# petitioner/MOAI-FHE-TransformerInference-Public

Hardware: AMD Instinct MI355X
Metric: NTT+INTT algorithmic GB/s (N=2^16, L=44x60-bit, batch=256 ciphertexts/GPU) vs HBM peak (higher is better)
Workload: dtype u64; 1 GPU; configs[1]: negacyclic NTT then INTT, N=65536, 44 x 60-bit primes, 256 ciphertexts x 2 polys per GPU; batch_per_gpu=256, batch_total=256, coeff_modulus=CoeffModulus::Create(65536, 44 x 60), bytes_per_coeff_per_transform=16

## Files before the change

moai-fhe-transformerinference-public_amd/csrc/launch.h:

```cpp
#pragma once
#include <type_traits>

#include "common.h"

namespace moai {

#define MOAI_KNOBS(X)                                                                                                          \
    X(NTT_FP, 1, "0: primes below 2^51 stay on the integer units in every transform, key switch and mod-down")                \
    X(NTT_LAZY8, 1, "0: integer primes below 2^60 take the exact butterflies instead of the approximate Shoup quotient")       \
    X(NTT_LDSTW, 1, "0: the forward contiguous pass loads its first stages' twiddles from memory instead of through LDS")      \
    X(NTT_CHUNK_MB, 0, "> 0: launch the two passes of a transform per chunk of polynomials of at most this many MiB")          \
    X(NTT_NAIVE, 0, "1: one launch per radix-2 stage over global memory (cross-check path)")                                   \
    X(NTT_COOP, 0, "1: the single-launch persistent transform (N >= 4096)")                                                    \
    X(NTT_COOP_WPC, 4, "single-launch transform: workgroups per compute unit")                                                 \
    X(NTT_COOP_DELAY, 4, "single-launch transform: rows a second pass stays behind the first")                                 \
    X(NTT_COOP_OCC, 4, "single-launch transform: occupancy the kernel is compiled for (3 or 4)")                               \
    X(KS_FP_MIN_ROWS, 16, "batch * L from which the key switch uses the FP64 arithmetic modes")                                \
    X(KS_TMP_MB, 8192, "MiB of key-switch digits in flight: sets how many output moduli share a launch")                       \
    X(KS_P1_ITEMS, 8, "1: the key switch's strided pass at N = 2^16 runs one tile per workgroup instead of eight, pipelined")  \
    X(KS_P1_PRE, 0, "1: the M_FPN strided pass of the key switch takes its twiddles as plain doubles")                         \
    X(KS_MAC_PF, 1, "key residues of the FP64 key-switch MAC: 0 loaded next to their use, 1 at its head, 2 at the digit's head") \
    X(KS_HOIST_PAIR, 4, "rotations per pass of the hoisted MAC in the FP64 modes: 4, 2, or 0 for one")                         \
    X(MD_FP_MIN_ROWS, 256, "polynomials * L from which mod-down and rescale use the FP64 arithmetic modes")                    \
    X(MATMUL_FP, 1, "0: moai_ct_pt_matmul keeps primes below 2^51 on the integer kernel")                                      \
    X(DEC_TMP_MB, 1024, "MiB of scratch per chunk of moai_ckks_decode when the stream's arena is smaller")

enum Knob
{
#define MOAI_KNOB_ID(id, dflt, what) K_##id,
    MOAI_KNOBS(MOAI_KNOB_ID)
#undef MOAI_KNOB_ID
    KNOB_COUNT
// ... 63 lines not shown
```

moai-fhe-transformerinference-public_amd/csrc/modarith.hip.h:

```cpp
#pragma once
#include "common.h"

namespace moai {

__device__ __forceinline__ uint64_t mulhi64(uint64_t a, uint64_t b)
{
    return __umul64hi(a, b);
}

__device__ __forceinline__ uint64_t mul_shoup_lazy(uint64_t y, uint64_t w, uint64_t wq, uint64_t q)
{
    uint64_t t = mulhi64(y, wq);
    return y * w + t * (0 - q);
}

__device__ __forceinline__ uint64_t csub(uint64_t x, uint64_t m)
{
    return x >= m ? x - m : x;
}

__device__ __forceinline__ uint64_t barrett128(uint64_t lo, uint64_t hi, uint64_t q, uint64_t cr0, uint64_t cr1)
{
    uint64_t carry = mulhi64(lo, cr0);
    uint64_t t_lo = lo * cr1;
// ... 77 lines not shown
__device__ __forceinline__ void fold2(uint64_t &lx, uint64_t &hx, uint64_t &ly, uint64_t &hy, uint64_t q, uint64_t cr0, uint64_t cr1)
{
    seed2(lx, hx, ly, hy, reduce2(lx, hx, ly, hy, q, cr0, cr1));
}

__device__ __forceinline__ void ct_bfly(uint64_t &x, uint64_t &y, uint64_t w, uint64_t wq, uint64_t q, uint64_t q2)
{
    uint64_t u = csub(x, q2);
    uint64_t v = mul_shoup_lazy(y, w, wq, q);
    x = u + v;
    y = u + q2 - v;
}

__device__ __forceinline__ void ct_bfly_noguard(uint64_t &x, uint64_t &y, uint64_t w, uint64_t wq, uint64_t q, uint64_t q2)
{
    uint64_t v = mul_shoup_lazy(y, w, wq, q);
    uint64_t u = x;
    x = u + v;
    y = u + q2 - v;
}

enum
{
    M_LAZY8 = -2,
    M_GUARD2 = -1,
    M_GUARD = 0,
    M_NOGUARD = 1,
    M_FPN = 2,
    M_FPR = 3
};

__device__ __forceinline__ double u2d(uint64_t b)
{
    return __longlong_as_double((long long)b);
}
__device__ __forceinline__ uint64_t d2u(double d)
{
    return (uint64_t)__double_as_longlong(d);
}
__device__ __forceinline__ double fp_from_u64(uint64_t v)
{
    return __builtin_fma((double)(uint32_t)(v >> 32), 4294967296.0, (double)(uint32_t)v);
}
__device__ __forceinline__ double fp_from_u52(uint64_t v)
{
    return u2d(v | 0x4330000000000000ull) - 4503599627370496.0;
// ... 91 lines not shown
    const uint32_t hi = (uint32_t)(p >> 32) + y0 * w1 + y1 * w0 + t0 * n1 + t1 * n0;
    return ((uint64_t)hi << 32) | (uint32_t)p;
}
__device__ __forceinline__ void ct_bfly_lazy8(uint64_t &x, uint64_t &y, uint64_t w, uint64_t wq, uint64_t nq, uint64_t n4q)
{
    const uint64_t u = csub_sign(x, n4q);
    const uint64_t v = mul_shoup_approx(y, w, wq, nq);
    x = u + v;
    y = u - (v + n4q);
}

__device__ __forceinline__ void gs_bfly_lazy8(uint64_t &x, uint64_t &y, uint64_t w, uint64_t wq, uint64_t nq, uint64_t n4q)
{
    const uint64_t u = x, v = y;
    x = csub_sign(u + v, n4q);
    y = mul_shoup_approx(u - (v + n4q), w, wq, nq);
}
__device__ __forceinline__ void gs_bfly_last_lazy8(uint64_t &x, uint64_t &y, const Tw &ninv, const Tw &ninv_w1, uint64_t nq, uint64_t n4q)
{
    const uint64_t u = x, v = y;
    x = mul_shoup_approx(u + v, ninv.w, ninv.wq, nq);
    y = mul_shoup_approx(u - (v + n4q), ninv_w1.w, ninv_w1.wq, nq);
}
template <bool LZ>
__device__ __forceinline__ void gs_bfly_sel(uint64_t &x, uint64_t &y, uint64_t w, uint64_t wq, uint64_t a, uint64_t b);

template <int MODE, int STAGES_LEFT = 0>
__device__ __forceinline__ void ct_bfly_t(uint64_t &x, uint64_t &y, uint64_t w, uint64_t wq, uint64_t q, uint64_t q2)
{
    if (MODE == M_LAZY8)
    {
        ct_bfly_lazy8(x, y, w, wq, q, q2);
    }
    else if (MODE == M_GUARD2)
    {
        ct_bfly_guard2<(STAGES_LEFT % 2) == 0>(x, y, w, wq, q, q2);
    }
    else if (MODE == M_FPN)
    {
        ct_bfly_fp<false>(x, y, w, wq, q, q2);
    }
    else if (MODE == M_FPR)
    {
        ct_bfly_fp<true>(x, y, w, wq, q, q2);
    }
    else if (MODE == M_NOGUARD)
// ... 83 lines not shown
```

moai-fhe-transformerinference-public_amd/csrc/ntt.hip:

```cpp
#include "ntt_kernels.hip.h"
#include "launch.h"

namespace moai {

bool noguard_ok(uint64_t q)
{
    return q < (~0ull) / 36;
}

int ntt_mode(const moai_ctx *c, uint32_t prime, bool allow_fp)
{
    const int m = (int)c->pc_host[prime].fp_mode;
    if (allow_fp && m && tuning(K_NTT_FP))
    {
        return m;
    }
    return noguard_ok(c->primes[prime]) ? M_NOGUARD : M_GUARD;
}

TwPair twiddles(const moai_ctx *c, int mode, bool inverse)
{
    if (mode >= M_FPN)
    {
        return inverse ? TwPair{ c->inv_twf, c->inv_twfb } : TwPair{ c->fwd_twf, c->fwd_twfb };
// ... 9 lines not shown
    a.tw = t.tw;
    a.twb = t.twb;
    a.pc = c->pc;
    a.rows = rows;
    for (size_t r = 0; r < MOAI_MAX_RNS; ++r)
    {
        a.sel.idx[r] = (uint32_t)(r < L ? r : 0);
        a.selp.idx[r] = rows.idx[r < L ? r : 0];
    }
    a.Lsel = (uint32_t)L;
    a.L = (uint32_t)L;
    a.n_poly = (uint32_t)n_poly;
    a.total_work = 0;
    a.src = nullptr;
    a.src_stride = a.src_off = 0;
    a.lds_twiddles = tuning(K_NTT_LDSTW) ? 1u : 0u;
    return a;
}

static bool lazy8_ok(const moai_ctx *c, uint32_t prime)
{
    return tuning(K_NTT_LAZY8) && c->primes[prime] < (1ull << 60);
}

template <int LOGN, int MODE>
static void launch_fwd_mode(const moai_ctx *c, NttArgs a, hipStream_t s)
{
    constexpr uint32_t tpr = 1u << (LOGN - 12);
    a.total_work = a.n_poly * a.Lsel * tpr;
    const TwPair t = twiddles(c, MODE, false);
    a.tw = t.tw;
    a.twb = t.twb;
    hipLaunchKernelGGL((ntt_fwd_strided<LOGN, MODE>), dim3(a.total_work), dim3(256), 0, s, a);
    hipLaunchKernelGGL((ntt_fwd_contig<LOGN, MODE>), dim3(a.total_work), dim3(256), 0, s, a);
}

template <int LOGN>
static int launch_fwd(const moai_ctx *c, const NttArgs &base, hipStream_t s)
{
    for (int mode : { M_LAZY8, M_GUARD2, M_NOGUARD, M_FPN, M_FPR })
    {
        NttArgs a = base;
        a.Lsel = 0;
        for (uint32_t r = 0; r < a.L; ++r)
        {
            const uint32_t prime = a.rows.idx[r];
            int m = ntt_mode(c, prime);
            if (m == M_GUARD)
            {
                m = lazy8_ok(c, prime) ? M_LAZY8 : M_GUARD2;
            }
            if (m == mode)
            {
                a.selp.idx[a.Lsel] = prime;
                a.sel.idx[a.Lsel++] = r;
            }
        }
        if (a.Lsel == 0)
        {
            continue;
        }
        MOAI_TRY((dispatch<M_LAZY8, M_GUARD2, M_NOGUARD, M_FPN, M_FPR>("forward transform mode ", mode, [&](auto MD) {
            launch_fwd_mode<LOGN, decltype(MD)::value>(c, a, s);
            return MOAI_OK;
        })));
    }
    return MOAI_OK;
}

template <int LOGN, int IM>
static void launch_inv_class(NttArgs a, hipStream_t s)
{
    constexpr uint32_t tpr = 1u << (LOGN - 12);
    if (!a.Lsel)
    {
        return;
    }
    a.total_work = a.n_poly * a.Lsel * tpr;
    hipLaunchKernelGGL((ntt_inv_contig<LOGN, IM>), dim3(a.total_work), dim3(256), 0, s, a);
    hipLaunchKernelGGL((ntt_inv_strided<LOGN, IM>), dim3(a.total_work), dim3(256), 0, s, a);
}

template <int LOGN>
static void launch_inv(const moai_ctx *c, const NttArgs &base, hipStream_t s)
{
    NttArgs cls[4] = { base, base, base, base };
    for (NttArgs &a : cls)
    {
        a.Lsel = 0;
    }
    const TwPair fp = twiddles(c, M_FPN, true);
    cls[2].tw = cls[3].tw = fp.tw;
    cls[2].twb = cls[3].twb = fp.twb;
    for (uint32_t r = 0; r < base.L; ++r)
    {
        const uint32_t prime = base.rows.idx[r];
        const int m = ntt_mode(c, prime);
        NttArgs &dst = m == M_FPN ? cls[2] : (m == M_FPR ? cls[3] : (lazy8_ok(c, prime) ? cls[1] : cls[0]));
        dst.selp.idx[dst.Lsel] = prime;
        dst.sel.idx[dst.Lsel++] = r;
    }
    launch_inv_class<LOGN, 0>(cls[0], s);
    launch_inv_class<LOGN, 1>(cls[1], s);
    launch_inv_class<LOGN, 2>(cls[2], s);
    launch_inv_class<LOGN, 3>(cls[3], s);
}

static size_t coop_grid(const moai_ctx *c)
{
    const long wpc = tuning(K_NTT_COOP_WPC);
    return (size_t)c->num_cu * (size_t)(wpc > 0 ? wpc : 4);
}

static uint32_t coop_delay()
{
    const long d = tuning(K_NTT_COOP_DELAY);
    return (uint32_t)(d > 0 ? d : 1);
}

static size_t coop_steps_cap(const moai_ctx *c, size_t rows)
{
    return rows + coop_delay() + coop_grid(c) + 8;
}

static size_t coop_state_bytes(const moai_ctx *c, size_t rows)
{
    return sizeof(CoopState) + sizeof(uint32_t) * (rows + 8 * coop_steps_cap(c, rows));
}
// ... 212 lines not shown
```

moai-fhe-transformerinference-public_amd/csrc/ntt_kernels.hip.h:

```cpp
#pragma once
#include "modarith.hip.h"

namespace moai {

__device__ __forceinline__ uint32_t xcd_remap(uint32_t b, uint32_t total)
{
    if (total & 7u)
    {
        return b;
    }
    return (b & 7u) * (total >> 3) + (b >> 3);
}

__device__ __forceinline__ void lds_barrier()
{
    asm volatile("s_waitcnt lgkmcnt(0)\n\ts_barrier" ::: "memory");
}

__device__ __forceinline__ void lds_wave_sync()
{
    asm volatile("s_waitcnt lgkmcnt(0)" ::: "memory");
}

__device__ __forceinline__ uint32_t phys_contig(uint32_t e)
// ... 12 lines not shown
    }
    return e;
}

struct NttArgs
{
    uint64_t *data;
    const Tw *tw;
    const Tw *twb;
    const PrimeConst *pc;
    RowMap rows;
    RowMap sel;
    RowMap selp;
    uint32_t L;
    uint32_t Lsel;
    uint32_t n_poly;
    uint32_t total_work;
    const uint64_t *src;
    uint32_t src_stride;
    uint32_t src_off;
    uint32_t lds_twiddles;
};

template <int MODE>
__device__ __forceinline__ uint64_t mode_q(const PrimeConst &pc)
{
    return MODE >= M_FPN ? pc.qd : (MODE == M_LAZY8 ? pc.nq : pc.q);
}
template <int MODE>
__device__ __forceinline__ uint64_t mode_q2(const PrimeConst &pc)
{
    return MODE >= M_FPN ? pc.qinv : (MODE == M_LAZY8 ? pc.n4q : pc.q2);
}

struct LoadIdentity
{
    __device__ __forceinline__ uint64_t operator()(uint64_t v) const
    {
        return v;
    }
};

struct LoadBarrett
{
    uint64_t q, cr1;
    __device__ __forceinline__ uint64_t operator()(uint64_t v) const
    {
        return barrett64(v, q, cr1);
    }
};

struct LoadFp
{
    uint64_t qd, qinv;
    __device__ __forceinline__ uint64_t operator()(uint64_t v) const
// ... 1 lines not shown
        return d2u(fp_red(fp_from_u64(v), u2d(qd), u2d(qinv)));
    }
};

struct LoadFp52
{
    uint64_t qd, qinv;
    __device__ __forceinline__ uint64_t operator()(uint64_t v) const
    {
        return d2u(fp_red(fp_from_u52(v), u2d(qd), u2d(qinv)));
    }
};

struct LoadBarrettFp
{
    uint64_t q, cr1, qd, qinv;
    __device__ __forceinline__ uint64_t operator()(uint64_t v) const
    {
        return d2u(fp_red(fp_from_u52(barrett64(v, q, cr1)), u2d(qd), u2d(qinv)));
    }
};


template <int MODE>
__device__ __forceinline__ void ct_bfly_stage(uint64_t &x, uint64_t &y, uint64_t w, uint64_t wq, uint64_t q, uint64_t q2, int stages_left)
{
    if (MODE == M_GUARD2)
    {
        if (stages_left & 1)
        {
            ct_bfly_guard2<false>(x, y, w, wq, q, q2);
        }
        else
        {
            ct_bfly_guard2<true>(x, y, w, wq, q, q2);
        }
    }
    else
    {
        ct_bfly_t<MODE>(x, y, w, wq, q, q2);
    }
}

template <int LOGN>
__device__ __forceinline__ void strided_load_raw(const uint64_t *__restrict__ irow, const uint32_t tid, uint64_t (&raw)[16])
{
    constexpr int GB = 12 - (LOGN - 8);
    constexpr uint32_t G = 1u << GB;
#pragma unroll
    for (int j = 0; j < 16; ++j)
// ... 10 lines not shown
{
    typedef const Tw __attribute__((address_space(4))) *TwConst;
    const TwConst twa = (TwConst)(uintptr_t)tw;
    constexpr int R1 = LOGN - 8;
    constexpr int RB = R1 - 4;
    constexpr int GB = 12 - R1;
    constexpr uint32_t G = 1u << GB;
#ifdef MOAI_DIAG_NOCOMPUTE
    const int diag_stages = (q == 0x7ff8dead0000beefull) ? 4 : 0;
#define MOAI_DIAG_STAGE_OK(u) && ((u) < diag_stages)
#else
#define MOAI_DIAG_STAGE_OK(u)
#endif
#pragma unroll
    for (int u = 0; u < 4; ++u)
    {
        const int half = 8 >> u;
#pragma unroll
        for (int j = 0; j < 16; ++j)
        {
            if (!(j & half) MOAI_DIAG_STAGE_OK(u))
            {
                const uint32_t ti = (1u << u) + (uint32_t)(j >> (4 - u));
                ct_bfly_stage<MODE>(x[j], x[j + half], twa[ti].w, twa[ti].wq, q, q2, LOGN - 1 - u);
            }
        }
    }
    if (RB > 0)
    {
        double twb[16];
        if (PRE)
        {
            const uint32_t thp = tid >> GB;
#pragma unroll
            for (int s = 4; s < R1; ++s)
            {
                const int cnt = 16 >> (R1 - s);
#pragma unroll
                for (int i = 0; i < cnt; ++i)
                {
                    twb[cnt - 1 + i] = tw1[(1u << s) + ((thp << (4 - (R1 - s))) | (uint32_t)i)];
                }
            }
        }
        if (SYNC_FIRST)
        {
            lds_barrier();
// ... 8 lines not shown
        const uint32_t th = tid >> GB;
#pragma unroll
        for (int j = 0; j < 16; ++j)
        {
            x[j] = lds[phys_strided<GB>((th << (GB + 4)) | ((uint32_t)j << GB) | g)];
        }
#pragma unroll
        for (int s = 4; s < R1; ++s)
        {
            const int half = 1 << (R1 - 1 - s);
#pragma unroll
            for (int j = 0; j < 16; ++j)
            {
                if (!(j & half) MOAI_DIAG_STAGE_OK(s - 4))
                {
                    if (PRE)
                    {
                        ct_bfly_fp1<MODE == M_FPR>(x[j], x[j + half], twb[(16 >> (R1 - s)) - 1 + (j >> (R1 - s))], u2d(q), u2d(q2));
                    }
                    else
                    {
                        uint32_t t_ = (th << 4) | (uint32_t)j;
                        Tw t = LDSTW ? ldstw[(1u << s) + (t_ >> (R1 - s))] : tw[(1u << s) + (t_ >> (R1 - s))];
                        ct_bfly_stage<MODE>(x[j], x[j + half], t.w, t.wq, q, q2, LOGN - 1 - s);
                    }
                }
            }
        }
#pragma unroll
        for (int j = 0; j < 16; ++j)
        {
            uint32_t t_ = (th << 4) | (uint32_t)j;
#ifdef MOAI_DIAG_NOSTORE
            if (x[j] == 0x7ff8dead0000beefull)
#endif
            row[(t_ << 8) + g] = x[j];
        }
    }
    else
    {
#pragma unroll
        for (int j = 0; j < 16; ++j)
        {
            uint32_t e = (uint32_t)j * 256u + tid;
            row[((e >> GB) << 8) + (e & (G - 1))] = x[j];
        }
    }
// ... 40 lines not shown
#pragma unroll 1
    for (uint32_t it = 0; it < (uint32_t)ITEMS; ++it)
    {
        uint32_t t = tid;
        asm volatile("" : "+v"(t));
        const bool more = it + 1u < (uint32_t)ITEMS;
        if (more)
        {
            strided_load_raw<LOGN>(inp + (tile0 + it + 1u) * G, t, raw);
        }
        strided_core<LOGN, MODE, false, true, true>(x, rowp + (tile0 + it) * G, tw, q, q2, lds, t, nullptr, ldstw);
        if (more)
        {
#pragma unroll
            for (int j = 0; j < 16; ++j)
            {
                x[j] = op(raw[j]);
            }
        }
    }
}

template <int LOGN, int MODE = M_GUARD>
__global__ __launch_bounds__(256, (MODE == M_GUARD2 || MODE == M_LAZY8 || MODE == M_FPR || MODE == M_NOGUARD) ? 4 : 5) void ntt_fwd_strided(NttArgs a)
{
    constexpr uint32_t TPR = 1u << (LOGN - 12);
    constexpr bool LDSTW = LOGN == 16 && (MODE == M_GUARD2 || MODE == M_LAZY8 || MODE == M_FPR || MODE == M_NOGUARD);
    __shared__ uint64_t lds[4096 + (LDSTW ? 512 : 0)];
    const uint32_t w = xcd_remap(blockIdx.x, a.total_work);
    const uint32_t tile = w % TPR;
    const uint32_t srow = w / TPR;
    const uint32_t si = srow % a.Lsel;
    const uint32_t r = __builtin_amdgcn_readfirstlane(a.sel.idx[si]);
    const uint32_t prime = __builtin_amdgcn_readfirstlane(a.selp.idx[si]);
    const PrimeConst &pc = a.pc[prime];
    uint64_t *rowp = a.data + ((size_t)((srow / a.Lsel) * a.L + r) << LOGN);
    if (MODE >= M_FPN)
    {
        LoadFp op;
        op.qd = pc.qd;
        op.qinv = pc.qinv;
        fwd_strided_tile<LOGN, LoadFp, MODE, false, LDSTW>(rowp, rowp, tile, a.tw + ((size_t)prime << LOGN), pc.qd, pc.qinv, lds, threadIdx.x, op);
    }
    else
    {
        fwd_strided_tile<LOGN, LoadIdentity, MODE, false, LDSTW>(rowp, rowp, tile, a.tw + ((size_t)prime << LOGN), mode_q<MODE>(pc), mode_q2<MODE>(pc),
                                                                 lds, threadIdx.x);
    }
}

struct StoreTile
{
    ulonglong2 *out;
    __device__ __forceinline__ void fetch(const uint32_t (&)[4])
    {
    }
    __device__ __forceinline__ void operator()(int, uint32_t ch, ulonglong2 v) const
    {
        out[ch] = v;
    }
};

template <int LOGN, int MODE = M_GUARD, class StoreOp = StoreTile>
__device__ __forceinline__ void fwd_contig_tile(uint64_t *__restrict__ rowp, uint32_t tile, const Tw *__restrict__ tw,
                                                uint64_t q, uint64_t q2, ulonglong2 *lds2, const uint32_t tid,
                                                const Tw *__restrict__ twb, uint64_t cr1, StoreOp store, Tw *ldstw = nullptr)
{
    constexpr int R1 = LOGN - 8;
    uint64_t *lds = reinterpret_cast<uint64_t *>(lds2);
    uint64_t *__restrict__ base = rowp + ((size_t)tile << 12);
    const uint32_t b = tid >> 4;
    const uint32_t tl = tid & 15u;
    const uint32_t blk = (tile << 4) + b;
    const Tw *__restrict__ twbt = twb + (size_t)tile * (15 * 256);

    if (ldstw)
    {
        const uint32_t lane = tid & 63u;
        if (lane < 60u)
        {
            const uint32_t bb = ((tid >> 6) << 2) + lane / 15u, i = lane % 15u;
            const uint32_t u = i == 0 ? 0u : (i < 3 ? 1u : (i < 7 ? 2u : 3u)), k = i - ((1u << u) - 1u);
            ldstw[bb * 15u + i] = tw[(1u << (R1 + u)) + (((tile << 4) + bb) << u) + k];
        }
    }
    uint64_t x[16];
#pragma unroll
    for (int j = 0; j < 16; ++j)
    {
        x[j] = base[(b << 8) | ((uint32_t)j << 4) | tl];
    }
    if (ldstw)
    {
        lds_wave_sync();
    }
#pragma unroll
    for (int u = 0; u < 4; ++u)
    {
        const int half = 8 >> u;
#pragma unroll
        for (int j = 0; j < 16; ++j)
        {
            if (!(j & half))
            {
                Tw t = ldstw ? ldstw[b * 15u + ((1u << u) - 1u) + (uint32_t)(j >> (4 - u))]
                             : tw[(1u << (R1 + u)) + (blk << u) + (uint32_t)(j >> (4 - u))];
                ct_bfly_stage<MODE>(x[j], x[j + half], t.w, t.wq, q, q2, 7 - u);
            }
        }
    }
#pragma unroll
    for (int j = 0; j < 16; ++j)
    {
        lds[phys_contig((b << 8) | ((uint32_t)j << 4) | tl)] = x[j];
    }
    lds_wave_sync();
    const uint32_t myrow = tid;
#pragma unroll
    for (int c = 0; c < 8; ++c)
    {
        ulonglong2 v = lds2[(myrow << 3) | ((uint32_t)c ^ (myrow & 7u))];
        x[2 * c] = v.x;
        x[2 * c + 1] = v.y;
    }
#pragma unroll
    for (int u = 4; u < 8; ++u)
    {
        const int half = 8 >> (u - 4);
#pragma unroll
        for (int j = 0; j < 16; ++j)
        {
            if (!(j & half))
            {
                Tw t = twbt[(((1u << (u - 4)) - 1u + (uint32_t)(j >> (8 - u))) << 8) + tid];
                ct_bfly_stage<MODE>(x[j], x[j + half], t.w, t.wq, q, q2, 7 - u);
            }
        }
    }
#pragma unroll
    for (int c = 0; c < 8; ++c)
    {
        ulonglong2 v;
        if (MODE >= M_FPN)
        {
            v.x = fp_to_canonical(u2d(x[2 * c]), u2d(q), u2d(q2));
            v.y = fp_to_canonical(u2d(x[2 * c + 1]), u2d(q), u2d(q2));
        }
        else if (MODE == M_NOGUARD)
        {
            v.x = barrett64(x[2 * c], q, cr1);
            v.y = barrett64(x[2 * c + 1], q, cr1);
        }
        else if (MODE == M_LAZY8)
        {
            const uint64_t n2q = (q2 >> 1) | 0x8000000000000000ull;
            v.x = csub_sign(csub_sign(csub_sign(x[2 * c], q2), n2q), q);
            v.y = csub_sign(csub_sign(csub_sign(x[2 * c + 1], q2), n2q), q);
        }
        else if (MODE == M_GUARD2)
        {
            v.x = csub(csub(csub(x[2 * c], q2 << 1), q2), q);
            v.y = csub(csub(csub(x[2 * c + 1], q2 << 1), q2), q);
        }
        else
        {
            v.x = csub(csub(x[2 * c], q2), q);
            v.y = csub(csub(x[2 * c + 1], q2), q);
        }
        lds2[(myrow << 3) | ((uint32_t)c ^ (myrow & 7u))] = v;
    }
    lds_wave_sync();
    const uint32_t wbase = (tid >> 6) << 9, lane = tid & 63u;
#pragma unroll
    for (int h = 0; h < 2; ++h)
    {
        uint32_t chs[4];
// ... 2 lines not shown
        {
            chs[i] = wbase + (uint32_t)(4 * h + i) * 64u + lane;
        }
        store.fetch(chs);
#pragma unroll
        for (int i = 0; i < 4; ++i)
        {
            const uint32_t rr = chs[i] >> 3;
            store(i, chs[i], lds2[(rr << 3) | ((chs[i] & 7u) ^ (rr & 7u))]);
        }
    }
}

template <int LOGN, int MODE = M_GUARD>
__device__ __forceinline__ void fwd_contig_tile(uint64_t *__restrict__ rowp, uint32_t tile, const Tw *__restrict__ tw,
                                                uint64_t q, uint64_t q2, ulonglong2 *lds2, const uint32_t tid,
                                                const Tw *__restrict__ twb, uint64_t cr1 = 0, Tw *ldstw = nullptr)
{
    StoreTile st;
    st.out = reinterpret_cast<ulonglong2 *>(rowp + ((size_t)tile << 12));
    fwd_contig_tile<LOGN, MODE, StoreTile>(rowp, tile, tw, q, q2, lds2, tid, twb, cr1, st, ldstw);
}

template <int LOGN, int MODE = M_GUARD>
__global__ __launch_bounds__(256) void ntt_fwd_contig(NttArgs a)
{
    constexpr uint32_t TPR = 1u << (LOGN - 12);
    __shared__ ulonglong2 lds2[2048 + 240];
    const uint32_t w = xcd_remap(blockIdx.x, a.total_work);
    const uint32_t pol = w % a.n_poly;
    const uint32_t rest = w / a.n_poly;
    const uint32_t tile = rest % TPR;
    const uint32_t r = __builtin_amdgcn_readfirstlane(a.sel.idx[rest / TPR]);
    const uint32_t prime = __builtin_amdgcn_readfirstlane(a.selp.idx[rest / TPR]);
    const PrimeConst &pc = a.pc[prime];
    fwd_contig_tile<LOGN, MODE>(a.data + (((size_t)pol * a.L + r) << LOGN), tile, a.tw + ((size_t)prime << LOGN),
                                mode_q<MODE>(pc), mode_q2<MODE>(pc), lds2, threadIdx.x,
                                a.twb + (size_t)prime * ((size_t)TPR * 15 * 256), pc.cr1, a.lds_twiddles ? reinterpret_cast<Tw *>(lds2 + 2048) : nullptr);
}

template <int LOGN, int IM = 0>
__device__ __forceinline__ void inv_contig_tile(uint64_t *rowp, uint32_t tile, const Tw *__restrict__ tw,
                                                uint64_t q, uint64_t q2, ulonglong2 *lds2, const uint32_t tid,
                                                const Tw *__restrict__ twb, const uint64_t *srcp = nullptr, Tw *ldstw = nullptr)
{
    constexpr int R1 = LOGN - 8;
    uint64_t *lds = reinterpret_cast<uint64_t *>(lds2);
    uint64_t *base = rowp + ((size_t)tile << 12);
    const uint32_t b = tid >> 4;
    const uint32_t tl = tid & 15u;
    const uint32_t blk = (tile << 4) + b;
    const Tw *__restrict__ twbt = twb + (size_t)tile * (15 * 256);

    Tw tb[15];
#pragma unroll
    for (int i = 0; i < 15; ++i)
    {
        tb[i] = twbt[((uint32_t)i << 8) + tid];
    }
    if (ldstw)
    {
        const uint32_t ln = tid & 63u;
        if (ln < 60u)
        {
            const uint32_t bb = ((tid >> 6) << 2) + ln / 15u, i = ln % 15u;
            const uint32_t u = i == 0 ? 0u : (i < 3 ? 1u : (i < 7 ? 2u : 3u)), k = i - ((1u << u) - 1u);
            ldstw[bb * 15u + i] = tw[(1u << (R1 + u)) + (((tile << 4) + bb) << u) + k];
        }
    }
    const ulonglong2 *in2 = reinterpret_cast<const ulonglong2 *>(srcp ? srcp + ((size_t)tile << 12) : base);
    const uint32_t wbase = (tid >> 6) << 9, lane = tid & 63u;
#pragma unroll
    for (int it = 0; it < 8; ++it)
    {
        uint32_t ch = wbase + (uint32_t)it * 64u + lane;
        uint32_t rr = ch >> 3;
        lds2[(rr << 3) | ((ch & 7u) ^ (rr & 7u))] = in2[ch];
    }
    lds_wave_sync();
    const uint32_t myrow = tid;
    uint64_t x[16];
#pragma unroll
    for (int c = 0; c < 8; ++c)
    {
        ulonglong2 v = lds2[(myrow << 3) | ((uint32_t)c ^ (myrow & 7u))];
        x[2 * c] = IM == 2 ? d2u(fp_red(fp_from_u52(v.x), u2d(q), u2d(q2))) : (IM == 3 ? d2u(fp_from_u52(v.x)) : v.x);
        x[2 * c + 1] = IM == 2 ? d2u(fp_red(fp_from_u52(v.y), u2d(q), u2d(q2))) : (IM == 3 ? d2u(fp_from_u52(v.y)) : v.y);
    }
#pragma unroll
    for (int u = 7; u >= 4; --u)
    {
        const int half = 8 >> (u - 4);
#pragma unroll
        for (int j = 0; j < 16; ++j)
        {
            if (!(j & half))
            {
                Tw t = tb[(1 << (u - 4)) - 1 + (j >> (8 - u))];
                gs_bfly_im<IM>(x[j], x[j + half], t.w, t.wq, q, q2, (u & 3) == 0);
            }
        }
    }
#pragma unroll
    for (int c = 0; c < 8; ++c)
    {
        ulonglong2 v;
        v.x = x[2 * c];
        v.y = x[2 * c + 1];
        lds2[(myrow << 3) | ((uint32_t)c ^ (myrow & 7u))] = v;
    }
    lds_wave_sync();
#pragma unroll
    for (int j = 0; j < 16; ++j)
    {
        x[j] = lds[phys_contig((b << 8) | ((uint32_t)j << 4) | tl)];
    }
#pragma unroll
    for (int u = 3; u >= 0; --u)
    {
        const int half = 8 >> u;
#pragma unroll
        for (int j = 0; j < 16; ++j)
        {
            if (!(j & half))
            {
                Tw t = ldstw ? ldstw[b * 15u + ((1u << u) - 1u) + (uint32_t)(j >> (4 - u))]
                             : tw[(1u << (R1 + u)) + (blk << u) + (uint32_t)(j >> (4 - u))];
                gs_bfly_im<IM>(x[j], x[j + half], t.w, t.wq, q, q2, (u & 3) == 0);
            }
        }
    }
#pragma unroll
    for (int j = 0; j < 16; ++j)
    {
        base[(b << 8) | ((uint32_t)j << 4) | tl] = x[j];
    }
}

template <int LOGN, int IM = 0>
__global__ __launch_bounds__(256) void ntt_inv_contig(NttArgs a)
{
    constexpr uint32_t TPR = 1u << (LOGN - 12);
    __shared__ ulonglong2 lds2[2048];
    const uint32_t w = xcd_remap(blockIdx.x, a.total_work);
    const uint32_t pol = w % a.n_poly;
    const uint32_t rest = w / a.n_poly;
    const uint32_t tile = rest % TPR;
    const uint32_t r = __builtin_amdgcn_readfirstlane(a.sel.idx[rest / TPR]);
    const uint32_t prime = __builtin_amdgcn_readfirstlane(a.selp.idx[rest / TPR]);
    const PrimeConst &pc = a.pc[prime];
    const uint64_t *srcp = a.src ? a.src + (((size_t)pol * a.src_stride + a.src_off + r) << LOGN) : nullptr;
    inv_contig_tile<LOGN, IM>(a.data + (((size_t)pol * a.L + r) << LOGN), tile, a.tw + ((size_t)prime << LOGN),
                              IM >= 2 ? pc.qd : (IM == 1 ? pc.nq : pc.q), IM >= 2 ? pc.qinv : (IM == 1 ? pc.n4q : pc.q2), lds2, threadIdx.x,
                              a.twb + (size_t)prime * ((size_t)TPR * 15 * 256), srcp);
}

template <int LOGN, int IM = 0>
__device__ __forceinline__ void inv_strided_tile(uint64_t *__restrict__ rowp, uint32_t tile, const Tw *__restrict__ tw,
                                                 const PrimeConst *pc, uint64_t *lds, const uint32_t tid)
{
    constexpr bool LZ = (IM == 1);
    constexpr int R1 = LOGN - 8;
    constexpr int RB = R1 - 4;
    constexpr int GB = 12 - R1;
    constexpr uint32_t G = 1u << GB;
    const uint64_t q = IM >= 2 ? pc->qd : (LZ ? pc->nq : pc->q);
    const uint64_t q2 = IM >= 2 ? pc->qinv : (LZ ? pc->n4q : pc->q2);
    uint64_t *__restrict__ row = rowp + tile * G;

    constexpr bool LDSTW = LOGN == 16 && IM == 1;
    Tw *ldstw = reinterpret_cast<Tw *>(lds + 4096);
    uint64_t x[16];
    if (RB > 0)
    {
        const uint32_t g = tid & (G - 1);
        const uint32_t th = tid >> GB;
        if (LDSTW)
        {
            ldstw[tid] = tw[tid];
        }
#pragma unroll
        for (int j = 0; j < 16; ++j)
        {
            uint32_t t_ = (th << 4) | (uint32_t)j;
            x[j] = row[(t_ << 8) + g];
        }
        if (LDSTW)
        {
            lds_barrier();
        }
#pragma unroll
        for (int s = R1 - 1; s >= 4; --s)
        {
            const int half = 1 << (R1 - 1 - s);
#pragma unroll
            for (int j = 0; j < 16; ++j)
            {
                if (!(j & half))
                {
                    uint32_t t_ = (th << 4) | (uint32_t)j;
                    Tw t = LDSTW ? ldstw[(1u << s) + (t_ >> (R1 - s))] : tw[(1u << s) + (t_ >> (R1 - s))];
                    gs_bfly_im<IM>(x[j], x[j + half], t.w, t.wq, q, q2, ((R1 - 1 - s) & 3) == 3);
                }
            }
        }
#pragma unroll
        for (int j = 0; j < 16; ++j)
        {
            lds[phys_strided<GB>((th << (GB + 4)) | ((uint32_t)j << GB) | g)] = x[j];
        }
        __syncthreads();
#pragma unroll
        for (int j = 0; j < 16; ++j)
        {
            x[j] = lds[phys_strided<GB>((uint32_t)j * 256u + tid)];
        }
    }
    else
    {
#pragma unroll
        for (int j = 0; j < 16; ++j)
        {
            uint32_t e = (uint32_t)j * 256u + tid;
            x[j] = row[((e >> GB) << 8) + (e & (G - 1))];
        }
    }
#pragma unroll
    for (int u = 3; u >= 1; --u)
    {
        const int half = 8 >> u;
#pragma unroll
        for (int j = 0; j < 16; ++j)
        {
            if (!(j & half))
            {
                Tw t = tw[(1u << u) + (uint32_t)(j >> (4 - u))];
                gs_bfly_im<IM>(x[j], x[j + half], t.w, t.wq, q, q2, ((RB + 3 - u) & 3) == 3);
            }
        }
    }
    {
        const Tw ninv = pc->ninv;
        const Tw ninv_w1 = pc->ninv_w1;
#pragma unroll
        for (int j = 0; j < 8; ++j)
        {
            if (IM >= 2)
            {
                gs_bfly_last_fp<IM == 3>(x[j], x[j + 8], fp_from_u64(ninv.w), fp_from_u64(ninv_w1.w), u2d(q), u2d(q2));
            }
            else if (LZ)
            {
                gs_bfly_last_lazy8(x[j], x[j + 8], ninv, ninv_w1, q, q2);
            }
            else
            {
                gs_bfly_last(x[j], x[j + 8], ninv, ninv_w1, q, q2);
            }
        }
    }
#pragma unroll
    for (int j = 0; j < 16; ++j)
    {
        uint32_t e = (uint32_t)j * 256u + tid;
        row[((e >> GB) << 8) + (e & (G - 1))] = IM >= 2 ? fp_to_canonical(u2d(x[j]), u2d(q), u2d(q2))
                                                        : (LZ ? csub_sign(csub_sign(x[j], (q2 >> 1) | 0x8000000000000000ull), q) : csub(x[j], q));
    }
}

template <int LOGN, int IM = 0>
__global__ __launch_bounds__(256, IM == 1 ? 4 : 5) void ntt_inv_strided(NttArgs a)
{
    constexpr uint32_t TPR = 1u << (LOGN - 12);
    __shared__ uint64_t lds[4096 + ((LOGN == 16 && IM == 1) ? 512 : 0)];
    const uint32_t w = xcd_remap(blockIdx.x, a.total_work);
    const uint32_t tile = w % TPR;
    const uint32_t srow = w / TPR;
    const uint32_t si = srow % a.Lsel;
    const uint32_t r = __builtin_amdgcn_readfirstlane(a.sel.idx[si]);
    const uint32_t prime = __builtin_amdgcn_readfirstlane(a.selp.idx[si]);
    inv_strided_tile<LOGN, IM>(a.data + ((size_t)((srow / a.Lsel) * a.L + r) << LOGN), tile, a.tw + ((size_t)prime << LOGN), a.pc + prime, lds,
                               threadIdx.x);
}

struct CoopState
{
    uint32_t next_row;
    uint32_t error;
    uint32_t pad0[30];
    struct
    {
        uint32_t head;
        uint32_t pad[31];
    } q[8];
};

struct CoopArgs
// ... 273 lines not shown
```

Before: 2229 GB/s.

## Add lazy-16q NTT butterflies with compile-time scheduled conditional subtractions

Adds an M_LAZY16 mode for 60-bit integer primes in which butterfly outputs may grow to 16q rather than 8q. A constexpr schedule decides at which stages a conditional subtraction is needed, so most stages skip the per-stage guard in both the forward and inverse passes. The forward contiguous kernel also gets a templated LDS twiddle fill that issues the global load before the data loads and writes LDS afterwards. This cuts integer ALU work per butterfly, at the cost of more kernel template instantiations and static bound checks that rely on the headroom of primes below 2^60.

New measurement: 2327 GB/s (median of 6 runs). +4.4%, better.

```diff
diff --git a/moai-fhe-transformerinference-public_amd/csrc/launch.h b/moai-fhe-transformerinference-public_amd/csrc/launch.h
--- a/moai-fhe-transformerinference-public_amd/csrc/launch.h
+++ b/moai-fhe-transformerinference-public_amd/csrc/launch.h
@@ -8,6 +8,7 @@
 #define MOAI_KNOBS(X)                                                                                                          \
     X(NTT_FP, 1, "0: primes below 2^51 stay on the integer units in every transform, key switch and mod-down")                \
     X(NTT_LAZY8, 1, "0: integer primes below 2^60 take the exact butterflies instead of the approximate Shoup quotient")       \
+    X(NTT_LAZY16, 1, "0: those primes keep values below 8q with a guard in every stage instead of below 16q with fewer (M_LAZY8)") \
     X(NTT_LDSTW, 1, "0: the forward contiguous pass loads its first stages' twiddles from memory instead of through LDS")      \
     X(NTT_CHUNK_MB, 0, "> 0: launch the two passes of a transform per chunk of polynomials of at most this many MiB")          \
     X(NTT_NAIVE, 0, "1: one launch per radix-2 stage over global memory (cross-check path)")                                   \
diff --git a/moai-fhe-transformerinference-public_amd/csrc/modarith.hip.h b/moai-fhe-transformerinference-public_amd/csrc/modarith.hip.h
--- a/moai-fhe-transformerinference-public_amd/csrc/modarith.hip.h
+++ b/moai-fhe-transformerinference-public_amd/csrc/modarith.hip.h
@@ -123,6 +123,7 @@
 
 enum
 {
+    M_LAZY16 = -3,
     M_LAZY8 = -2,
     M_GUARD2 = -1,
     M_GUARD = 0,
@@ -260,6 +261,118 @@
     x = mul_shoup_approx(u + v, ninv.w, ninv.wq, nq);
     y = mul_shoup_approx(u - (v + n4q), ninv_w1.w, ninv_w1.wq, nq);
 }
+__device__ __forceinline__ uint64_t csub_carry(uint64_t x, uint64_t neg_m)
+{
+    const uint64_t d = x + neg_m;
+    return d < x ? d : x;
+}
+struct Lazy16Fwd
+{
+    uint32_t g8, g4;
+    int end;
+    int peak;
+};
+constexpr Lazy16Fwd lazy16_fwd(int logn, int first, int count, int b0)
+{
+    Lazy16Fwd r{ 0, 0, b0, b0 };
+    int b = b0;
+    for (int s = first; s < first + count; ++s)
+    {
+        int u = b;
+        if (s == logn - 1)
+        {
+            if (u > 8)
+            {
+                r.g8 |= 1u << s;
+                u = u - 8 > 8 ? u - 8 : 8;
+            }
+            if (u > 4)
+            {
+                r.g4 |= 1u << s;
+                u = u - 4 > 4 ? u - 4 : 4;
+            }
+        }
+        else if (b + 4 > 16)
+        {
+            r.g8 |= 1u << s;
+            u = b - 8 > 8 ? b - 8 : 8;
+        }
+        b = u + 4;
+        r.peak = b > r.peak ? b : r.peak;
+    }
+    r.end = b;
+    return r;
+}
+constexpr int lazy16_fwd_handover(int logn)
+{
+    return (logn & 1) ? 12 : 16;
+}
+template <int G>
+__device__ __forceinline__ void ct_bfly_lazy16(uint64_t &x, uint64_t &y, uint64_t w, uint64_t wq, uint64_t nq, uint64_t n4q)
+{
+    uint64_t u = x;
+    if (G & 1)
+    {
+        u = csub_carry(u, n4q << 1);
+    }
+    if (G & 2)
+    {
+        u = csub_carry(u, n4q);
+    }
+    const uint64_t v = mul_shoup_approx(y, w, wq, nq);
+    x = u + v;
+    y = u - (v + n4q);
+}
+struct Lazy16Inv
+{
+    uint32_t xk;
+    int out;
+    int peak;
+};
+constexpr Lazy16Inv lazy16_inv(int count, int bin, bool last)
+{
+    Lazy16Inv r{ 0, bin, bin };
+    int bx = bin;
+    for (int i = 0; i < count; ++i)
+    {
+        const bool fin = last && i == count - 1;
+        const int sum = 2 * bx;
+        if (bx > 4)
+        {
+            r.xk |= 1u << i;
+            r.peak = bx > 8 ? 99 : r.peak;
+        }
+        r.peak = sum > r.peak ? sum : r.peak;
+        const int xout = fin ? 4 : (sum > 8 ? (sum - 8 > 8 ? sum - 8 : 8) : sum);
+        const int pout = (i > 0 && !fin) ? 8 : 4;
+        bx = xout > pout ? xout : pout;
+    }
+    r.out = bx;
+    return r;
+}
+constexpr int lazy16_inv_handover()
+{
+    return 8;
+}
+template <int K>
+__device__ __forceinline__ void gs_bfly_lazy16(uint64_t &x, uint64_t &y, uint64_t w, uint64_t wq, uint64_t nq, uint64_t n4q)
+{
+    const uint64_t u = x, v = y;
+    x = K ? csub_carry(u + v, n4q << 1) : u + v;
+    y = mul_shoup_approx(u - (v + (K ? n4q << 1 : n4q)), w, wq, nq);
+}
+template <int K>
+__device__ __forceinline__ void gs_bfly_last_lazy16(uint64_t &x, uint64_t &y, const Tw &ninv, const Tw &ninv_w1, uint64_t nq, uint64_t n4q)
+{
+    const uint64_t u = x, v = y;
+    x = mul_shoup_approx(u + v, ninv.w, ninv.wq, nq);
+    y = mul_shoup_approx(u - (v + (K ? n4q << 1 : n4q)), ninv_w1.w, ninv_w1.wq, nq);
+}
+__device__ __forceinline__ int lazy16_inv_kind(uint32_t xk, int i, int j, int half)
+{
+    return (i > 0 && (j & (half >> 1))) ? 0 : (int)((xk >> i) & 1u);
+}
+
 template <bool LZ>
 __device__ __forceinline__ void gs_bfly_sel(uint64_t &x, uint64_t &y, uint64_t w, uint64_t wq, uint64_t a, uint64_t b);
 
diff --git a/moai-fhe-transformerinference-public_amd/csrc/ntt.hip b/moai-fhe-transformerinference-public_amd/csrc/ntt.hip
--- a/moai-fhe-transformerinference-public_amd/csrc/ntt.hip
+++ b/moai-fhe-transformerinference-public_amd/csrc/ntt.hip
@@ -55,6 +55,10 @@
 {
     return tuning(K_NTT_LAZY8) && c->primes[prime] < (1ull << 60);
 }
+static bool lazy16_ok(const moai_ctx *c, uint32_t prime)
+{
+    return lazy8_ok(c, prime) && tuning(K_NTT_LAZY16);
+}
 
 template <int LOGN, int MODE>
 static void launch_fwd_mode(const moai_ctx *c, NttArgs a, hipStream_t s)
@@ -65,13 +69,27 @@
     a.tw = t.tw;
     a.twb = t.twb;
     hipLaunchKernelGGL((ntt_fwd_strided<LOGN, MODE>), dim3(a.total_work), dim3(256), 0, s, a);
-    hipLaunchKernelGGL((ntt_fwd_contig<LOGN, MODE>), dim3(a.total_work), dim3(256), 0, s, a);
+    if constexpr (MODE == M_LAZY16)
+    {
+        if (a.lds_twiddles)
+        {
+            hipLaunchKernelGGL((ntt_fwd_contig<LOGN, MODE, 1>), dim3(a.total_work), dim3(256), 0, s, a);
+        }
+        else
+        {
+            hipLaunchKernelGGL((ntt_fwd_contig<LOGN, MODE, 0>), dim3(a.total_work), dim3(256), 0, s, a);
+        }
+    }
+    else
+    {
+        hipLaunchKernelGGL((ntt_fwd_contig<LOGN, MODE>), dim3(a.total_work), dim3(256), 0, s, a);
+    }
 }
 
 template <int LOGN>
 static int launch_fwd(const moai_ctx *c, const NttArgs &base, hipStream_t s)
 {
-    for (int mode : { M_LAZY8, M_GUARD2, M_NOGUARD, M_FPN, M_FPR })
+    for (int mode : { M_LAZY16, M_LAZY8, M_GUARD2, M_NOGUARD, M_FPN, M_FPR })
     {
         NttArgs a = base;
         a.Lsel = 0;
@@ -81,7 +99,7 @@
             int m = ntt_mode(c, prime);
             if (m == M_GUARD)
             {
-                m = lazy8_ok(c, prime) ? M_LAZY8 : M_GUARD2;
+                m = lazy16_ok(c, prime) ? M_LAZY16 : (lazy8_ok(c, prime) ? M_LAZY8 : M_GUARD2);
             }
             if (m == mode)
             {
@@ -93,7 +111,7 @@
         {
             continue;
         }
-        MOAI_TRY((dispatch<M_LAZY8, M_GUARD2, M_NOGUARD, M_FPN, M_FPR>("forward transform mode ", mode, [&](auto MD) {
+        MOAI_TRY((dispatch<M_LAZY16, M_LAZY8, M_GUARD2, M_NOGUARD, M_FPN, M_FPR>("forward transform mode ", mode, [&](auto MD) {
             launch_fwd_mode<LOGN, decltype(MD)::value>(c, a, s);
             return MOAI_OK;
         })));
@@ -117,7 +135,7 @@
 template <int LOGN>
 static void launch_inv(const moai_ctx *c, const NttArgs &base, hipStream_t s)
 {
-    NttArgs cls[4] = { base, base, base, base };
+    NttArgs cls[5] = { base, base, base, base, base };
     for (NttArgs &a : cls)
     {
         a.Lsel = 0;
@@ -129,7 +147,7 @@
     {
         const uint32_t prime = base.rows.idx[r];
         const int m = ntt_mode(c, prime);
-        NttArgs &dst = m == M_FPN ? cls[2] : (m == M_FPR ? cls[3] : (lazy8_ok(c, prime) ? cls[1] : cls[0]));
+        NttArgs &dst = m == M_FPN ? cls[2] : (m == M_FPR ? cls[3] : (lazy16_ok(c, prime) ? cls[4] : (lazy8_ok(c, prime) ? cls[1] : cls[0])));
         dst.selp.idx[dst.Lsel] = prime;
         dst.sel.idx[dst.Lsel++] = r;
     }
@@ -137,6 +155,7 @@
     launch_inv_class<LOGN, 1>(cls[1], s);
     launch_inv_class<LOGN, 2>(cls[2], s);
     launch_inv_class<LOGN, 3>(cls[3], s);
+    launch_inv_class<LOGN, IM_LAZY16>(cls[4], s);
 }
 
 static size_t coop_grid(const moai_ctx *c)
diff --git a/moai-fhe-transformerinference-public_amd/csrc/ntt_kernels.hip.h b/moai-fhe-transformerinference-public_amd/csrc/ntt_kernels.hip.h
--- a/moai-fhe-transformerinference-public_amd/csrc/ntt_kernels.hip.h
+++ b/moai-fhe-transformerinference-public_amd/csrc/ntt_kernels.hip.h
@@ -58,15 +58,21 @@
     uint32_t lds_twiddles;
 };
 
+constexpr bool mode_lazy(int mode)
+{
+    return mode == M_LAZY8 || mode == M_LAZY16;
+}
+constexpr int IM_LAZY16 = -1;
+
 template <int MODE>
 __device__ __forceinline__ uint64_t mode_q(const PrimeConst &pc)
 {
-    return MODE >= M_FPN ? pc.qd : (MODE == M_LAZY8 ? pc.nq : pc.q);
+    return MODE >= M_FPN ? pc.qd : (mode_lazy(MODE) ? pc.nq : pc.q);
 }
 template <int MODE>
 __device__ __forceinline__ uint64_t mode_q2(const PrimeConst &pc)
 {
-    return MODE >= M_FPN ? pc.qinv : (MODE == M_LAZY8 ? pc.n4q : pc.q2);
+    return MODE >= M_FPN ? pc.qinv : (mode_lazy(MODE) ? pc.n4q : pc.q2);
 }
 
 struct LoadIdentity
@@ -114,10 +120,37 @@
 };
 
 
-template <int MODE>
+template <int MODE, int LOGN = 0>
 __device__ __forceinline__ void ct_bfly_stage(uint64_t &x, uint64_t &y, uint64_t w, uint64_t wq, uint64_t q, uint64_t q2, int stages_left)
 {
-    if (MODE == M_GUARD2)
+    if constexpr (MODE == M_LAZY16)
+    {
+        constexpr int R1 = LOGN - 8;
+        constexpr Lazy16Fwd p1 = lazy16_fwd(LOGN, 0, R1, 8), p2 = lazy16_fwd(LOGN, R1, 8, lazy16_fwd_handover(LOGN));
+        static_assert(p1.peak <= 16 && p2.peak <= 16, "a value of 16q or more");
+        static_assert(p1.end == lazy16_fwd_handover(LOGN), "the contiguous pass starts from another bound");
+        static_assert(p2.end <= 8, "the final subtractions expect values below 8q");
+        constexpr uint32_t g8 = p1.g8 | p2.g8, g4 = p1.g4 | p2.g4;
+        const int s = LOGN - 1 - stages_left;
+        const int g = (int)((g8 >> s) & 1u) | ((int)((g4 >> s) & 1u) << 1);
+        if (g == 0)
+        {
+            ct_bfly_lazy16<0>(x, y, w, wq, q, q2);
+        }
+        else if (g == 1)
+        {
+            ct_bfly_lazy16<1>(x, y, w, wq, q, q2);
+        }
+        else if (g == 2)
+        {
+            ct_bfly_lazy16<2>(x, y, w, wq, q, q2);
+        }
+        else
+        {
+            ct_bfly_lazy16<3>(x, y, w, wq, q, q2);
+        }
+    }
+    else if (MODE == M_GUARD2)
     {
         if (stages_left & 1)
         {
@@ -174,7 +207,7 @@
             if (!(j & half) MOAI_DIAG_STAGE_OK(u))
             {
                 const uint32_t ti = (1u << u) + (uint32_t)(j >> (4 - u));
-                ct_bfly_stage<MODE>(x[j], x[j + half], twa[ti].w, twa[ti].wq, q, q2, LOGN - 1 - u);
+                ct_bfly_stage<MODE, LOGN>(x[j], x[j + half], twa[ti].w, twa[ti].wq, q, q2, LOGN - 1 - u);
             }
         }
     }
@@ -229,7 +262,7 @@
                     {
                         uint32_t t_ = (th << 4) | (uint32_t)j;
                         Tw t = LDSTW ? ldstw[(1u << s) + (t_ >> (R1 - s))] : tw[(1u << s) + (t_ >> (R1 - s))];
-                        ct_bfly_stage<MODE>(x[j], x[j + half], t.w, t.wq, q, q2, LOGN - 1 - s);
+                        ct_bfly_stage<MODE, LOGN>(x[j], x[j + half], t.w, t.wq, q, q2, LOGN - 1 - s);
                     }
                 }
             }
@@ -316,10 +349,10 @@
 }
 
 template <int LOGN, int MODE = M_GUARD>
-__global__ __launch_bounds__(256, (MODE == M_GUARD2 || MODE == M_LAZY8 || MODE == M_FPR || MODE == M_NOGUARD) ? 4 : 5) void ntt_fwd_strided(NttArgs a)
+__global__ __launch_bounds__(256, (MODE == M_GUARD2 || mode_lazy(MODE) || MODE == M_FPR || MODE == M_NOGUARD) ? 4 : 5) void ntt_fwd_strided(NttArgs a)
 {
     constexpr uint32_t TPR = 1u << (LOGN - 12);
-    constexpr bool LDSTW = LOGN == 16 && (MODE == M_GUARD2 || MODE == M_LAZY8 || MODE == M_FPR || MODE == M_NOGUARD);
+    constexpr bool LDSTW = LOGN == 16 && (MODE == M_GUARD2 || mode_lazy(MODE) || MODE == M_FPR || MODE == M_NOGUARD);
     __shared__ uint64_t lds[4096 + (LDSTW ? 512 : 0)];
     const uint32_t w = xcd_remap(blockIdx.x, a.total_work);
     const uint32_t tile = w % TPR;
@@ -355,7 +388,7 @@
     }
 };
 
-template <int LOGN, int MODE = M_GUARD, class StoreOp = StoreTile>
+template <int LOGN, int MODE = M_GUARD, class StoreOp = StoreTile, int TWL = -1>
 __device__ __forceinline__ void fwd_contig_tile(uint64_t *__restrict__ rowp, uint32_t tile, const Tw *__restrict__ tw,
                                                 uint64_t q, uint64_t q2, ulonglong2 *lds2, const uint32_t tid,
                                                 const Tw *__restrict__ twb, uint64_t cr1, StoreOp store, Tw *ldstw = nullptr)
@@ -368,10 +401,21 @@
     const uint32_t blk = (tile << 4) + b;
     const Tw *__restrict__ twbt = twb + (size_t)tile * (15 * 256);
 
-    if (ldstw)
+    const bool use_lds = TWL < 0 ? ldstw != nullptr : TWL == 1;
+    Tw fill;
+    uint32_t fill_slot = 0;
+    if (use_lds)
     {
         const uint32_t lane = tid & 63u;
-        if (lane < 60u)
+        if (TWL == 1)
+        {
+            const uint32_t l = lane < 59u ? lane : 59u;
+            const uint32_t bb = ((tid >> 6) << 2) + l / 15u, i = l % 15u;
+            const uint32_t u = i == 0 ? 0u : (i < 3 ? 1u : (i < 7 ? 2u : 3u)), k = i - ((1u << u) - 1u);
+            fill = tw[(1u << (R1 + u)) + (((tile << 4) + bb) << u) + k];
+            fill_slot = bb * 15u + i;
+        }
+        else if (lane < 60u)
         {
             const uint32_t bb = ((tid >> 6) << 2) + lane / 15u, i = lane % 15u;
             const uint32_t u = i == 0 ? 0u : (i < 3 ? 1u : (i < 7 ? 2u : 3u)), k = i - ((1u << u) - 1u);
@@ -384,8 +428,12 @@
     {
         x[j] = base[(b << 8) | ((uint32_t)j << 4) | tl];
     }
-    if (ldstw)
-    {
+    if (use_lds)
+    {
+        if (TWL == 1 && (tid & 63u) < 60u)
+        {
+            ldstw[fill_slot] = fill;
+        }
         lds_wave_sync();
     }
 #pragma unroll
@@ -397,9 +445,9 @@
         {
             if (!(j & half))
             {
-                Tw t = ldstw ? ldstw[b * 15u + ((1u << u) - 1u) + (uint32_t)(j >> (4 - u))]
-                             : tw[(1u << (R1 + u)) + (blk << u) + (uint32_t)(j >> (4 - u))];
-                ct_bfly_stage<MODE>(x[j], x[j + half], t.w, t.wq, q, q2, 7 - u);
+                Tw t = use_lds ? ldstw[b * 15u + ((1u << u) - 1u) + (uint32_t)(j >> (4 - u))]
+                               : tw[(1u << (R1 + u)) + (blk << u) + (uint32_t)(j >> (4 - u))];
+                ct_bfly_stage<MODE, LOGN>(x[j], x[j + half], t.w, t.wq, q, q2, 7 - u);
             }
         }
     }
@@ -427,7 +475,7 @@
             if (!(j & half))
             {
                 Tw t = twbt[(((1u << (u - 4)) - 1u + (uint32_t)(j >> (8 - u))) << 8) + tid];
-                ct_bfly_stage<MODE>(x[j], x[j + half], t.w, t.wq, q, q2, 7 - u);
+                ct_bfly_stage<MODE, LOGN>(x[j], x[j + half], t.w, t.wq, q, q2, 7 - u);
             }
         }
     }
@@ -445,7 +493,7 @@
             v.x = barrett64(x[2 * c], q, cr1);
             v.y = barrett64(x[2 * c + 1], q, cr1);
         }
-        else if (MODE == M_LAZY8)
+        else if (mode_lazy(MODE))
         {
             const uint64_t n2q = (q2 >> 1) | 0x8000000000000000ull;
             v.x = csub_sign(csub_sign(csub_sign(x[2 * c], q2), n2q), q);
@@ -494,7 +542,7 @@
     fwd_contig_tile<LOGN, MODE, StoreTile>(rowp, tile, tw, q, q2, lds2, tid, twb, cr1, st, ldstw);
 }
 
-template <int LOGN, int MODE = M_GUARD>
+template <int LOGN, int MODE = M_GUARD, int TWL = -1>
 __global__ __launch_bounds__(256) void ntt_fwd_contig(NttArgs a)
 {
     constexpr uint32_t TPR = 1u << (LOGN - 12);
@@ -506,9 +554,33 @@
     const uint32_t r = __builtin_amdgcn_readfirstlane(a.sel.idx[rest / TPR]);
     const uint32_t prime = __builtin_amdgcn_readfirstlane(a.selp.idx[rest / TPR]);
     const PrimeConst &pc = a.pc[prime];
-    fwd_contig_tile<LOGN, MODE>(a.data + (((size_t)pol * a.L + r) << LOGN), tile, a.tw + ((size_t)prime << LOGN),
-                                mode_q<MODE>(pc), mode_q2<MODE>(pc), lds2, threadIdx.x,
-                                a.twb + (size_t)prime * ((size_t)TPR * 15 * 256), pc.cr1, a.lds_twiddles ? reinterpret_cast<Tw *>(lds2 + 2048) : nullptr);
+    uint64_t *rowp = a.data + (((size_t)pol * a.L + r) << LOGN);
+    StoreTile st;
+    st.out = reinterpret_cast<ulonglong2 *>(rowp + ((size_t)tile << 12));
+    fwd_contig_tile<LOGN, MODE, StoreTile, TWL>(rowp, tile, a.tw + ((size_t)prime << LOGN), mode_q<MODE>(pc), mode_q2<MODE>(pc), lds2, threadIdx.x,
+                                                a.twb + (size_t)prime * ((size_t)TPR * 15 * 256), pc.cr1, st,
+                                                (TWL < 0 ? a.lds_twiddles != 0 : TWL == 1) ? reinterpret_cast<Tw *>(lds2 + 2048) : nullptr);
+}
+
+template <int IM>
+__device__ __forceinline__ void gs_bfly_tile(uint64_t (&x)[16], int j, int half, uint64_t w, uint64_t wq, uint64_t q, uint64_t q2, const bool redsum,
+                                             uint32_t xk, int i)
+{
+    if (IM == IM_LAZY16)
+    {
+        if (lazy16_inv_kind(xk, i, j, half))
+        {
+            gs_bfly_lazy16<1>(x[j], x[j + half], w, wq, q, q2);
+        }
+        else
+        {
+            gs_bfly_lazy16<0>(x[j], x[j + half], w, wq, q, q2);
+        }
+    }
+    else
+    {
+        gs_bfly_im<IM>(x[j], x[j + half], w, wq, q, q2, redsum);
+    }
 }
 
 template <int LOGN, int IM = 0>
@@ -523,6 +595,9 @@
     const uint32_t tl = tid & 15u;
     const uint32_t blk = (tile << 4) + b;
     const Tw *__restrict__ twbt = twb + (size_t)tile * (15 * 256);
+    constexpr Lazy16Inv z1 = lazy16_inv(4, 4, false), z2 = lazy16_inv(4, z1.out, false);
+    static_assert(z1.peak <= 16 && z2.peak <= 16, "a value of 16q or more");
+    static_assert(z2.out == lazy16_inv_handover(), "the strided pass starts from another bound");
 
     Tw tb[15];
 #pragma unroll
@@ -569,7 +644,7 @@
             if (!(j & half))
             {
                 Tw t = tb[(1 << (u - 4)) - 1 + (j >> (8 - u))];
-                gs_bfly_im<IM>(x[j], x[j + half], t.w, t.wq, q, q2, (u & 3) == 0);
+                gs_bfly_tile<IM>(x, j, half, t.w, t.wq, q, q2, (u & 3) == 0, z1.xk, 7 - u);
             }
         }
     }
@@ -598,7 +673,7 @@
             {
                 Tw t = ldstw ? ldstw[b * 15u + ((1u << u) - 1u) + (uint32_t)(j >> (4 - u))]
                              : tw[(1u << (R1 + u)) + (blk << u) + (uint32_t)(j >> (4 - u))];
-                gs_bfly_im<IM>(x[j], x[j + half], t.w, t.wq, q, q2, (u & 3) == 0);
+                gs_bfly_tile<IM>(x, j, half, t.w, t.wq, q, q2, (u & 3) == 0, z2.xk, 3 - u);
             }
         }
     }
@@ -622,8 +697,9 @@
     const uint32_t prime = __builtin_amdgcn_readfirstlane(a.selp.idx[rest / TPR]);
     const PrimeConst &pc = a.pc[prime];
     const uint64_t *srcp = a.src ? a.src + (((size_t)pol * a.src_stride + a.src_off + r) << LOGN) : nullptr;
+    constexpr bool LZ = IM == 1 || IM == IM_LAZY16;
     inv_contig_tile<LOGN, IM>(a.data + (((size_t)pol * a.L + r) << LOGN), tile, a.tw + ((size_t)prime << LOGN),
-                              IM >= 2 ? pc.qd : (IM == 1 ? pc.nq : pc.q), IM >= 2 ? pc.qinv : (IM == 1 ? pc.n4q : pc.q2), lds2, threadIdx.x,
+                              IM >= 2 ? pc.qd : (LZ ? pc.nq : pc.q), IM >= 2 ? pc.qinv : (LZ ? pc.n4q : pc.q2), lds2, threadIdx.x,
                               a.twb + (size_t)prime * ((size_t)TPR * 15 * 256), srcp);
 }
 
@@ -631,7 +707,7 @@
 __device__ __forceinline__ void inv_strided_tile(uint64_t *__restrict__ rowp, uint32_t tile, const Tw *__restrict__ tw,
                                                  const PrimeConst *pc, uint64_t *lds, const uint32_t tid)
 {
-    constexpr bool LZ = (IM == 1);
+    constexpr bool LZ = (IM == 1 || IM == IM_LAZY16);
     constexpr int R1 = LOGN - 8;
     constexpr int RB = R1 - 4;
     constexpr int GB = 12 - R1;
@@ -639,8 +715,11 @@
     const uint64_t q = IM >= 2 ? pc->qd : (LZ ? pc->nq : pc->q);
     const uint64_t q2 = IM >= 2 ? pc->qinv : (LZ ? pc->n4q : pc->q2);
     uint64_t *__restrict__ row = rowp + tile * G;
-
-    constexpr bool LDSTW = LOGN == 16 && IM == 1;
+    constexpr Lazy16Inv zb = lazy16_inv(RB, lazy16_inv_handover(), false), za = lazy16_inv(4, zb.out, true);
+    static_assert(zb.peak <= 16 && za.peak <= 16, "a value of 16q or more");
+    static_assert(za.out <= 4, "the final subtractions expect values below 4q");
+
+    constexpr bool LDSTW = LOGN == 16 && LZ;
     Tw *ldstw = reinterpret_cast<Tw *>(lds + 4096);
     uint64_t x[16];
     if (RB > 0)
@@ -672,7 +751,7 @@
                 {
                     uint32_t t_ = (th << 4) | (uint32_t)j;
                     Tw t = LDSTW ? ldstw[(1u << s) + (t_ >> (R1 - s))] : tw[(1u << s) + (t_ >> (R1 - s))];
-                    gs_bfly_im<IM>(x[j], x[j + half], t.w, t.wq, q, q2, ((R1 - 1 - s) & 3) == 3);
+                    gs_bfly_tile<IM>(x, j, half, t.w, t.wq, q, q2, ((R1 - 1 - s) & 3) == 3, zb.xk, R1 - 1 - s);
                 }
             }
         }
@@ -707,7 +786,7 @@
             if (!(j & half))
             {
                 Tw t = tw[(1u << u) + (uint32_t)(j >> (4 - u))];
-                gs_bfly_im<IM>(x[j], x[j + half], t.w, t.wq, q, q2, ((RB + 3 - u) & 3) == 3);
+                gs_bfly_tile<IM>(x, j, half, t.w, t.wq, q, q2, ((RB + 3 - u) & 3) == 3, za.xk, 3 - u);
             }
         }
     }
@@ -717,7 +796,18 @@
 #pragma unroll
         for (int j = 0; j < 8; ++j)
         {
-            if (IM >= 2)
+            if (IM == IM_LAZY16)
+            {
+                if (lazy16_inv_kind(za.xk, 3, j, 8))
+                {
+                    gs_bfly_last_lazy16<1>(x[j], x[j + 8], ninv, ninv_w1, q, q2);
+                }
+                else
+                {
+                    gs_bfly_last_lazy16<0>(x[j], x[j + 8], ninv, ninv_w1, q, q2);
+                }
+            }
+            else if (IM >= 2)
             {
                 gs_bfly_last_fp<IM == 3>(x[j], x[j + 8], fp_from_u64(ninv.w), fp_from_u64(ninv_w1.w), u2d(q), u2d(q2));
             }
@@ -741,10 +831,10 @@
 }
 
 template <int LOGN, int IM = 0>
-__global__ __launch_bounds__(256, IM == 1 ? 4 : 5) void ntt_inv_strided(NttArgs a)
+__global__ __launch_bounds__(256, (IM == 1 || IM == IM_LAZY16) ? 4 : 5) void ntt_inv_strided(NttArgs a)
 {
     constexpr uint32_t TPR = 1u << (LOGN - 12);
-    __shared__ uint64_t lds[4096 + ((LOGN == 16 && IM == 1) ? 512 : 0)];
+    __shared__ uint64_t lds[4096 + ((LOGN == 16 && (IM == 1 || IM == IM_LAZY16)) ? 512 : 0)];
     const uint32_t w = xcd_remap(blockIdx.x, a.total_work);
     const uint32_t tile = w % TPR;
     const uint32_t srow = w / TPR;
```
